# reesque/SfmFromScratch

Measured on AMD Instinct MI355X. Metric: images/sec detect+describe+match, 1080p, 1/2/4/8 MI355X, higher is better.
Workload: dtype f32; 1 GPU; BASELINE configs[1]: 32x 1080p per GPU, ScaleRotInvSIFT 4-level x2 octave pyramid, k=2500, fw 18, NNRatio 0.85 over consecutive pairs; frames_per_gpu=32, pairs_per_gpu=31, distinct_batches=2, parallelism=image-shard x1, batches_in_flight=2

## Files before the change

### include/sfmfeat.h

```cpp
#ifndef SFMFEAT_H_
#define SFMFEAT_H_

#include <stddef.h>
#include <stdint.h>

#ifdef __cplusplus
extern "C" {
#endif

#define SFM_OK 0
#define SFM_EINVAL 1
#define SFM_ESTATE 2
#define SFM_EDEVICE 3
#define SFM_ERANGE 4
#define SFM_EINDEX 5

#define SFM_MODE_SCALEROT 0
#define SFM_MODE_NAIVE 1

#define SFM_DESC_DIM 128
#define SFM_MAX_GAUSS 15
#define SFM_MAX_KSIZE 31
#define SFM_MAX_FW 64
#define SFM_MAX_LEVELS 12
// ... 221 lines not shown

int32_t sfm_debug_nms(int32_t device, const float* R, int32_t B, int32_t H, int32_t W, int32_t ksize,
                      const uint32_t* tnms, int32_t tile, uint64_t* keys_out, int64_t* counts_out);

#define SFM_SELECT_STATE_WORDS 11
#define SFM_SELECT_CONSTS 5
int32_t sfm_debug_select(int32_t device, int32_t nlevels, int32_t B, const float* const* R, const int32_t* H,
                         const int32_t* W, const int32_t* half_window, int32_t k, int32_t ksize, int64_t vmin,
                         int32_t force_exact, int32_t* x, int32_t* y, float* conf, int32_t* count,
                         uint32_t* state, int64_t* ncand, int32_t* consts);

float sfm_debug_time_harris(int32_t device, int32_t abl, int32_t B, int32_t H, int32_t W,
                            int32_t iters);
float sfm_debug_harris_stamps(int32_t device, int32_t abl, int32_t B, int32_t H, int32_t W,
                              int32_t iters, uint64_t* out, int64_t cap);

int64_t sfm_debug_match_stamps(uint64_t* out, int64_t cap);

int32_t sfm_debug_match_operands(sfm_ctx* ctx, int32_t slot, int64_t rows, uint16_t* hi, uint16_t* lo,
                                 float* norm2, float* rnorm, float* pmax);
int32_t sfm_debug_match_windows(sfm_ctx* ctx, int32_t pair, int64_t rows, int32_t* cand_n, float* cand_thr,
                                uint32_t* cand);
int32_t sfm_debug_match_skips(sfm_ctx* ctx, int32_t pair, int64_t rows, uint8_t* skip);

int32_t sfm_copy_wg(void* dst, const void* src, int64_t bytes, int32_t workgroups, void* stream);

int32_t sfm_debug_select_stats(sfm_ctx* ctx, int32_t* fallback_planes, int32_t* total_planes);
int32_t sfm_debug_pose_candidates(sfm_ctx* ctx, int32_t* cand_idx, int64_t entries);
int32_t sfm_debug_ransac_fits(sfm_ctx* ctx, double* F, int32_t* counts, int64_t entries);
int32_t sfm_debug_pnp_fits(sfm_ctx* ctx, double* hyp, int32_t* counts, double* start_Rt, int64_t entries);
int32_t sfm_debug_copy_level(sfm_ctx* ctx, int32_t l, int32_t what, float* out, void* stream);
int64_t sfm_debug_bmax_stride(int32_t h, int32_t w);
void sfm_debug_set_nms_blocks(int32_t mode);
int32_t sfm_debug_nms_blocks_rule(int32_t h, int32_t w, int32_t kcap, int32_t ksize);
int32_t sfm_debug_nms_blocks(int32_t device, const float* R, int32_t B, int32_t H, int32_t W, const uint32_t* tnms,
                             const uint32_t* fallback, int32_t blocks, int32_t inflate, uint64_t* keys_out,
                             int64_t* counts_out);


#ifdef __cplusplus
}
#endif

#endif
```

### sfmfromscratch_amd/_native.py

```python
from __future__ import annotations

import ctypes
import os
import sys
import threading

import numpy as np

from . import _abi
from ._abi import SfmParams

_HERE = os.path.dirname(os.path.abspath(__file__))
LIB_PATH = os.environ.get("SFMFEAT_LIB", os.path.join(_HERE, "lib", "libsfmfeat.so"))

_lib = None
_lib_lock = threading.Lock()

_fp = ctypes.POINTER(ctypes.c_float)
_i64p = ctypes.POINTER(ctypes.c_int64)
_i32p = ctypes.POINTER(ctypes.c_int32)
_u8p = ctypes.POINTER(ctypes.c_uint8)
_dp = ctypes.POINTER(ctypes.c_double)
_vp = ctypes.c_void_p

# ... 78 lines not shown
    "sfm_gate_destroy": (ctypes.c_int32, [_vp]),
    "sfm_ctx_set_gate": (ctypes.c_int32, [_vp, _vp]),
    "sfm_profile_enable": (ctypes.c_int32, [_vp, ctypes.c_int32]),
    "sfm_profile_stages": (ctypes.c_int32, [_vp, ctypes.c_int32]),
    "sfm_profile_read": (ctypes.c_int32, [_vp, ctypes.POINTER(ctypes.c_double), _i64p, ctypes.c_int32]),
    "sfm_profile_spans": (ctypes.c_int32, [_vp, ctypes.c_int64]),
    "sfm_profile_spans_read": (ctypes.c_int32, [_vp, _i64p, _i32p, ctypes.c_int64, _i64p, _i64p, ctypes.c_int32]),
    "sfm_debug_time_harris": (ctypes.c_float, [ctypes.c_int32] * 6),
    "sfm_debug_harris_stamps": (ctypes.c_float, [ctypes.c_int32] * 6 + [ctypes.c_void_p, ctypes.c_int64]),
    "sfm_debug_match_stamps": (ctypes.c_int64, [ctypes.c_void_p, ctypes.c_int64]),
    "sfm_debug_select_stats": (ctypes.c_int32, [_vp, _i32p, _i32p]),
    **_abi.MATCH_DEBUG_SIGNATURES,
    **_abi.GEOM_DEBUG_SIGNATURES,
    **_abi.SELECT_DEBUG_SIGNATURES,
    **_abi.PNP_DEBUG_SIGNATURES,
    "sfm_copy_wg": (ctypes.c_int32, [_vp, _vp, ctypes.c_int64, ctypes.c_int32, _vp]),
    "sfm_dist_unique_id": (ctypes.c_int32, [_u8p]),
    "sfm_dist_create": (ctypes.c_int32, [ctypes.c_int32, ctypes.c_int32, ctypes.c_int32, _u8p, ctypes.POINTER(_vp)]),
    "sfm_dist_destroy": (ctypes.c_int32, [_vp]),
    "sfm_dist_last_error": (ctypes.c_char_p, [_vp]),
    "sfm_dist_rank": (ctypes.c_int32, [_vp, _i32p, _i32p]),
    "sfm_dist_allgather_slots_dev": (ctypes.c_int32, [_vp, ctypes.c_int32, ctypes.c_int32, _vp, _vp, _vp, _vp, _vp,
                                                      _vp, ctypes.c_int64, _vp]),
    "sfm_dist_halo_dev": (ctypes.c_int32, [_vp, ctypes.c_int32, _vp, _vp, _vp, _vp, _vp, _vp, _vp]),

    "sfm_debug_copy_level": (ctypes.c_int32, [_vp, ctypes.c_int32, ctypes.c_int32, _vp, _vp]),
    "sfm_debug_atan2": (ctypes.c_int32, [ctypes.c_int32, _fp, _fp, _fp, ctypes.c_int64]),
    "sfm_debug_harris": (ctypes.c_int32, [ctypes.c_int32, _fp, ctypes.c_int32, ctypes.c_double, ctypes.c_int32,
                                          _fp, ctypes.c_int32, ctypes.c_int32, _fp, _fp, _i64p]),
    "sfm_debug_nms": (ctypes.c_int32, [ctypes.c_int32, _fp, ctypes.c_int32, ctypes.c_int32, ctypes.c_int32,
                                       ctypes.c_int32, _vp, ctypes.c_int32, _vp, _i64p]),
    "sfm_debug_bmax_stride": (ctypes.c_int64, [ctypes.c_int32, ctypes.c_int32]),
    "sfm_debug_set_nms_blocks": (None, [ctypes.c_int32]),
    "sfm_debug_nms_blocks_rule": (ctypes.c_int32, [ctypes.c_int32] * 4),
    "sfm_debug_nms_blocks": (ctypes.c_int32, [ctypes.c_int32, _fp, ctypes.c_int32, ctypes.c_int32, ctypes.c_int32,
                                              _vp, _vp, ctypes.c_int32, ctypes.c_int32, _vp, _i64p]),
}


class NativeLibraryMissing(ImportError):
    pass


def _preload_torch_hip_runtime():
    import importlib.util
    spec = importlib.util.find_spec("torch")
    if spec is None or not spec.submodule_search_locations:
        return
    for d in spec.submodule_search_locations:
        cand = os.path.join(d, "lib", "libamdhip64.so")
        if os.path.exists(cand):
            try:
                ctypes.CDLL(cand, mode=ctypes.RTLD_GLOBAL)
            except OSError:
                pass
            return


def _preload_torch_rccl():
    import importlib.util
    if "torch" not in sys.modules and importlib.util.find_spec("torch") is not None:
        import torch


def load_library(path: str | None = None):
    global _lib
# ... 444 lines not shown
    nc = ctypes.c_int64(0)
    check(load_library().sfm_debug_harris(device, g.ctypes.data_as(_fp), gs, params.alpha, params.ksize,
                                          img.ctypes.data_as(_fp), H, W, R.ctypes.data_as(_fp),
                                          med.ctypes.data_as(_fp), ctypes.byref(nc)))
    return R, med[0], nc.value


def debug_nms(R: np.ndarray, tnms, ksize: int = 3, tile: bool = False, device: int = 0):
    R = np.ascontiguousarray(R, dtype=np.float32)
    B, H, W = R.shape
    t = np.ascontiguousarray(tnms, dtype=np.uint32)
    keys = np.zeros(B * H * W, np.uint64)
    cnt = np.zeros(B, np.int64)
    check(load_library().sfm_debug_nms(device, R.ctypes.data_as(_fp), B, H, W, ksize, t.ctypes.data,
                                       int(tile), keys.ctypes.data, cnt.ctypes.data_as(_i64p)))
    return [np.sort(keys[b * H * W: b * H * W + cnt[b]]) for b in range(B)]


def debug_nms_blocks(R: np.ndarray, tnms, fallback=None, blocks: bool = True, inflate: bool = False, device: int = 0):
    R = np.ascontiguousarray(R, dtype=np.float32)
    B, H, W = R.shape
    t = np.ascontiguousarray(tnms, dtype=np.uint32)
    fb = np.zeros(B, np.uint32) if fallback is None else np.ascontiguousarray(fallback, dtype=np.uint32)
    assert t.shape == (B,) and fb.shape == (B,)
    keys = np.zeros(B * H * W, np.uint64)
    cnt = np.zeros(B, np.int64)
    check(load_library().sfm_debug_nms_blocks(device, R.ctypes.data_as(_fp), B, H, W, t.ctypes.data, fb.ctypes.data,
                                              int(blocks), int(inflate), keys.ctypes.data, cnt.ctypes.data_as(_i64p)))
    return [np.sort(keys[b * H * W: b * H * W + cnt[b]]) for b in range(B)]


def set_nms_blocks(mode: int):
    load_library().sfm_debug_set_nms_blocks(int(mode))


def nms_blocks_rule(h: int, w: int, kcap: int, ksize: int = 3) -> bool:
    return bool(load_library().sfm_debug_nms_blocks_rule(int(h), int(w), int(kcap), int(ksize)))


def bmax_stride(h: int, w: int) -> int:
    return int(load_library().sfm_debug_bmax_stride(int(h), int(w)))


def debug_geom(op: int, rows: np.ndarray, device: int = 0) -> np.ndarray:
    op = int(op)
    if not 0 <= op < len(_abi.GEOM_ROW_IN):
        raise ValueError(f"debug_geom: unknown op {op}")
    if not isinstance(rows, np.ndarray) or rows.dtype != np.float64 or not rows.flags.c_contiguous:
        raise ValueError("debug_geom: rows must be a C-contiguous float64 array")
    if rows.ndim != 2 or rows.shape[1] != _abi.GEOM_ROW_IN[op]:
        raise ValueError(f"debug_geom: op {op} takes rows of {_abi.GEOM_ROW_IN[op]} values, got shape {rows.shape}")
    n = rows.shape[0]
    if n > _abi.SFM_GEOM_MAX_ROWS:
        raise ValueError(f"debug_geom: at most {_abi.SFM_GEOM_MAX_ROWS} rows")
    out = np.empty((n, _abi.GEOM_ROW_OUT[op]), np.float64)
    if n:
        check(load_library().sfm_debug_geom(device, op, rows.ctypes.data, n, out.ctypes.data))
    return out


def select_constants(k: int) -> dict:
    consts = np.zeros(_abi.SFM_SELECT_CONSTS, np.int32)
    check(load_library().sfm_debug_select(0, 0, 0, None, None, None, None, int(k), 1, 0, 0, None, None, None, None,
                                          None, None, consts.ctypes.data))
    return dict(zip(_abi.SELECT_CONST_FIELDS, consts.tolist()))

# ... 147 lines not shown
```

### sfmfromscratch_amd/csrc/api_extract.hip

```cpp
#include "ctx.h"

using namespace sfm;

static_assert(kLayoutMedBins == kMedBins1 && kLayoutCounterStride == kCounterStride &&
                  kLayoutMedianStateBytes == sizeof(MedianState) && kLayoutSelectMaxLevels == kSelectMaxLevels,
              "extract_layout.h mirrors kernels.h");
static_assert(layout_bmax_stride(1080, 1920) == bmax_plane_stride(1080, 1920) &&
                  layout_bmax_stride(270, 480) == bmax_plane_stride(270, 480) &&
                  layout_bmax_stride(70, 132) == bmax_plane_stride(70, 132),
              "extract_layout.h mirrors kernels.h");

static int g_nms_blocks_override = -2;
void extract_set_nms_blocks(int mode) { g_nms_blocks_override = mode < -1 ? -2 : mode; }

LayoutSwitches extract_layout_switches() {
  LayoutSwitches s = extract_switches().layout;
  if (g_nms_blocks_override != -2) s.nms_blocks = g_nms_blocks_override;
  return s;
}

const ExtractSwitches& extract_switches() {
  static const ExtractSwitches sw = [] {
    ExtractSwitches s;
    s.layout.pyr_fused = env_int(getenv("SFMFEAT_PYR_FUSED"), 1) != 0;
    s.layout.exact_px = env_int(getenv("SFMFEAT_EXACT_PX"), 128);
    s.layout.select_merge = env_int(SFM_DIAG_ENV("SFMFEAT_SELECT_MERGE"), 1) != 0;
    s.layout.nms_blocks = env_int(SFM_DIAG_ENV("SFMFEAT_NMS_BLOCKS"), -1);
    s.fill_launches = env_int(SFM_DIAG_ENV("SFMFEAT_FILL_LAUNCHES"), 0) != 0;
    s.harris_group = env_int(SFM_DIAG_ENV("SFMFEAT_HARRIS_GROUP"), 0);
    s.gate_level = env_int(SFM_DIAG_ENV("SFMFEAT_GATE_LEVEL"), 0);
    s.select_caller = env_int(SFM_DIAG_ENV("SFMFEAT_SELECT_CALLER"), 0) == 1;
    s.skip = env_int(SFM_ABLATION_ENV("SFMFEAT_SKIP"), 0);
    return s;
  }();
  return sw;
}

namespace {

int layout_of(sfm_ctx* c, int B, int H, int W, ExtractLayout* y) {
  if (extract_layout(&c->p, c->kcap, B, H, W, c->serial, extract_layout_switches(), y) != SFM_OK)
    return set_err(c, SFM_EINVAL, "image too small for the pyramid");
  return SFM_OK;
}

int reserve(sfm_ctx* c, const ExtractLayout& y) {
  for (int i = 0; i < kExtractBufs; ++i)
    if (int rc = ensure(c, c->ex.buf[i], y.bytes[i])) return rc;
  return SFM_OK;
}

struct Extraction {
  sfm_ctx* c;
  const ExtractSwitches& sw;
  const ExtractLayout& y;
  int B, skip;
  hipStream_t st;
  int32_t* xy;
  float* desc;
  float* conf;
  int32_t* count;
  int64_t cap;
  MatchOperands mo;
  const float* lvl[SFM_MAX_LEVELS];
// ... 51 lines not shown
      q.scan = SelectScan{med(l), medcnt + y.counter[l], donecnt + y.counter[l], vmin, exact(l) ? 1 : 0};
      q.down[0] = q.down[1] = q.down[2] = nullptr;
      if (y.pyr_fused && l == 0)
        for (int k = 0; k < 3; ++k) q.down[k] = const_cast<float*>(lvl[1 + k]);
    }
    if (l1 - l0 == 1 && y.bmax[l0] >= 0 && ((uintptr_t)R(l0) & 15) == 0 &&
        nms_blocks_shape(y.lv[l0].w, c->p.ksize, 0) &&
        (extract_layout_switches().nms_blocks == 1 || harris_tiles_64(g, B, c->p.gaussian_size))) {
      g.l[0].bmax = bmax(l0);
      mapped[l0] = true;
      c->ex.last_mapped |= 1u << l0;
    }
    ProfilerWs& pr = c->prof;
    if (pr.span_cap > 0) {
      if (pr.span_n < pr.span_cap) {
        g.span = as<unsigned long long>(pr.spans) + 2 * pr.span_n++;
        pr.span_level.push_back(l0);
      } else {
        ++pr.span_dropped;
      }
    }
    const float alpha = (float)c->p.alpha;
    if (!(l0 > 0 && (skip & 16))) launch_harris_levels(g, B, as<float>(c->ex.gauss), c->p.gaussian_size, alpha, st);
  }

  void select_level(int l, hipStream_t s) {
    StageScope sc(c, SFM_PROF_TOPK, s);
    if (skip & 1) return;
    launch_select(R(l), cand(l), candcnt + y.counter[l], at<uint32_t>(kBufMedlist, y.sel[l]),
                  at<uint64_t>(kBufScratch, y.sel[l]), kp(l), std::max(c->kcap, 1), c->kcap, B, y.lv[l].h, y.lv[l].w,
                  c->p.ksize, y.lv[l].fw / 2, med(l), s);
  }

  void select_merged() {
    StageScope sc(c, SFM_PROF_TOPK, st);
    SelectLevels g{};
    g.n = y.L - y.L_aux;
    for (int l = y.L_aux; l < y.L; ++l)
      g.l[l - y.L_aux] = SelectLevels::Level{R(l), cand(l), candcnt + y.counter[l], at<uint32_t>(kBufMedlist, y.sel[l]),
                                             at<uint64_t>(kBufScratch, y.sel[l]), kp(l), med(l), y.lv[l].h, y.lv[l].w,
                                             y.lv[l].fw / 2};
    if (!(skip & 1)) launch_select_levels(g, std::max(c->kcap, 1), c->kcap, B, c->p.ksize, st);
  }

  void describe_level(int l, hipStream_t s) {
    StageScope sc(c, SFM_PROF_DESCRIBE, s);
    const int L = y.L;
    if ((skip & 2) && l != L - 1) {
      fused_ok = false;
      return;
    }
    bool ow = false;
    const bool r = launch_describe(lvl[l], B, y.lv[l].h, y.lv[l].w, y.lv[l].fw, c->p.mode == SFM_MODE_NAIVE ? 0 : 1,
                                   kp(l), c->kcap, as<int32_t>(c->ex.buf[kBufLc]), l, L, y.lv[l].scale, xy, desc, conf,
                                   cap, l == L - 1 ? count : nullptr, mo, &ow, s);
    if (l == L - 1) counted = r;
    fused_ok = fused_ok && ow;
  }

  int release_gate() {
    if (c->gate && !gate_released) {
      HIPCHK(c, hipEventRecord(c->gate->ev, st));
      c->gate->armed = true;
      gate_released = true;
    }
    return SFM_OK;
  }

  int run(const float* imgs);
};

int Extraction::run(const float* imgs) {
  const int L = y.L, L_aux = y.L_aux;
  CtxStreams& cs = c->s;
  int rc;
  lvl[0] = imgs;
  for (int l = 1; l < L; ++l) lvl[l] = at<float>(kBufLvl, y.lvl[l]);
  zeroed = sw.fill_launches;
  {
    StageScope sc(c, SFM_PROF_PYRAMID, st);
    if (!y.pyr_fused) pyramid_from(1);
  }
  if ((rc = operands_fused_begin(c, desc, count, cap, B, &mo))) return rc;
  if (mo.hi) HIPCHK(c, hipMemsetAsync(mo.pmax, 0, (size_t)B * match_pmax_bytes(mo.capP), st));
  fused_ok = mo.hi != nullptr;
  if (!zeroed || sw.fill_launches) {
    HIPCHK(c, hipMemsetAsync(c->ex.buf[kBufHist].p, 0, y.bytes[kBufHist], st));
    HIPCHK(c, hipMemsetAsync(c->ex.buf[kBufCounts].p, 0, y.bytes[kBufCounts], st));
    zeroed = true;
  }
  medcnt = as<unsigned long long>(c->ex.buf[kBufCounts]);
  candcnt = medcnt + y.counter_block;
  donecnt = medcnt + 3 * y.counter_block;
  hipStream_t ax = nullptr;
  if (L_aux > 0) {
    if (!cs.aux) HIPCHK(c, hipStreamCreateWithPriority(&cs.aux, hipStreamNonBlocking, cs.prio));
    ax = cs.aux;
    HIPCHK(c, hipEventRecord(cs.ev[L], st));
    HIPCHK(c, hipStreamWaitEvent(ax, cs.ev[L], 0));
  }
  for (int l0 = 0; l0 < L;) {
    int l1 = l0 + 1;
    if (sw.harris_group > 0 && l0 >= sw.harris_group) l1 = std::min(L, l0 + kHarrisMaxLevels);
    harris(l0, l1);
    if (y.pyr_fused && l0 == 0 && L > 4) {
      StageScope sc(c, SFM_PROF_PYRAMID, st);
      pyramid_from(4);
    }
    if (sw.gate_level >= l0 && sw.gate_level < l1 && (rc = release_gate())) return rc;
    for (int l = l0; l < l1; ++l) {
      if (!exact(l)) {
        StageScope sc(c, SFM_PROF_NMS, st);
        launch_nms(R(l), med(l), cand(l), candcnt + y.counter[l], B, y.lv[l].h, y.lv[l].w, c->p.ksize, 0, st, 0,
                   mapped[l] ? bmax(l) : nullptr);
      }
      if (l < L_aux) {
        if (sw.select_caller) select_level(l, st);
        HIPCHK(c, hipEventRecord(cs.ev[l], st));
        HIPCHK(c, hipStreamWaitEvent(ax, cs.ev[l], 0));
        if (!sw.select_caller) select_level(l, ax);
        if (l == L_aux - 1) HIPCHK(c, hipEventRecord(cs.ev[L + 2], ax));
        describe_level(l, ax);
      }
    }
    l0 = l1;
  }
  if ((rc = release_gate())) return rc;
  if (y.select_merged) {
    select_merged();
  } else {
    for (int l = L_aux; l < L; ++l) select_level(l, st);
  }
  if (L_aux > 0 && L > L_aux) HIPCHK(c, hipStreamWaitEvent(st, cs.ev[L + 2], 0));
  for (int l = L_aux; l < L; ++l) describe_level(l, st);
  if (L_aux > 0) {
    HIPCHK(c, hipEventRecord(cs.ev[L + 1], ax));
    HIPCHK(c, hipStreamWaitEvent(st, cs.ev[L + 1], 0));
  }
  if (!counted) launch_finalize_counts(as<int32_t>(c->ex.buf[kBufLc]), B, L, count, st);
  HIPCHK(c, hipGetLastError());
  if (fused_ok && counted) operands_fused_commit(c, B);
  return SFM_OK;
}

}

int extract_reserve(sfm_ctx* c, int B, int H, int W) {
  ExtractLayout y;
  if (int rc = layout_of(c, B, H, W, &y)) return rc;
  return reserve(c, y);
}

int extract_impl(sfm_ctx* c, const float* imgs, int B, int H, int W, int32_t* xy, float* desc, float* conf,
                 int32_t* count, int64_t cap, hipStream_t st) {
  if (B < 1 || H < 1 || W < 1) return set_err(c, SFM_EINVAL, "empty batch or image");
  if (cap < c->cap) return set_err(c, SFM_ERANGE, "slot capacity below L * int(k / L)");
  ExtractLayout y;
  int rc;
  if ((rc = layout_of(c, B, H, W, &y)) || (rc = reserve(c, y))) return rc;
  const ExtractSwitches& sw = extract_switches();
  ExtractWs& x = c->ex;
  const int skip = x.extractions++ > 0 ? sw.skip : 0;
  if (c->gate && c->gate->armed) HIPCHK(c, hipStreamWaitEvent(st, c->gate->ev, 0));
  x.last_B = B;
  x.last_H = H;
  x.last_W = W;
  x.last_mapped = 0;
// ... 79 lines not shown
```

### sfmfromscratch_amd/csrc/ctx.h

```cpp
#pragma once

#include <stdlib.h>
#include <string.h>

#include <algorithm>
#include <string>
#include <utility>
#include <vector>

#include "../../include/sfmfeat.h"
#include "extract_layout.h"
#include "kernels.h"

struct DevBuf {
  void* p = nullptr;
  size_t bytes = 0;
  DevBuf() = default;
  DevBuf(const DevBuf&) = delete;
  DevBuf& operator=(const DevBuf&) = delete;
  DevBuf(DevBuf&& o) noexcept : p(o.p), bytes(o.bytes) { o.p = nullptr, o.bytes = 0; }
  DevBuf& operator=(DevBuf&& o) noexcept {
    if (this != &o) {
      release();
      std::swap(p, o.p);
// ... 195 lines not shown
  hipStream_t st;
  hipEvent_t a = nullptr, b = nullptr;
  static hipEvent_t event(ProfilerWs& pr) {
    hipEvent_t e = nullptr;
    if (pr.pool.empty()) {
      (void)hipEventCreate(&e);
    } else {
      e = pr.pool.back();
      pr.pool.pop_back();
    }
    return e;
  }
  StageScope(sfm_ctx* c, int stage_, hipStream_t st_) : pr(c->prof), stage(stage_), st(st_) {
    if (pr.on && ((pr.mask >> stage) & 1u)) {
      a = event(pr);
      b = event(pr);
      (void)hipEventRecord(a, st);
    }
  }
  ~StageScope() {
    if (a) {
      (void)hipEventRecord(b, st);
      pr.pending.push_back({stage, {a, b}});
    }
  }
};

struct ExtractSwitches {
  sfm::LayoutSwitches layout;
  bool fill_launches;
  int harris_group;
  int gate_level;
  bool select_caller;
  int skip;
};
const ExtractSwitches& extract_switches();
sfm::LayoutSwitches extract_layout_switches();
void extract_set_nms_blocks(int mode);

int extract_reserve(sfm_ctx* c, int B, int H, int W);
int extract_impl(sfm_ctx* c, const float* imgs, int B, int H, int W, int32_t* xy, float* desc, float* conf,
                 int32_t* count, int64_t cap, hipStream_t st);

const std::vector<int32_t>& ransac_stream(sfm_ctx* c, int n, int iters);

int operands_fused_begin(sfm_ctx* c, const float* desc, const int32_t* count, int64_t cap, int B,
                         sfm::MatchOperands* mo);
void operands_fused_commit(sfm_ctx* c, int B);
void operands_fused_clear(sfm_ctx* c);
```

### sfmfromscratch_amd/csrc/debug_nms.hip

```cpp
#include <math.h>
#include <string.h>

#include <vector>

#include "ctx.h"

using namespace sfm;

extern "C" {

int64_t sfm_debug_bmax_stride(int32_t h, int32_t w) { return bmax_plane_stride(h, w); }

void sfm_debug_set_nms_blocks(int32_t mode) { extract_set_nms_blocks(mode); }

int32_t sfm_debug_nms_blocks_rule(int32_t h, int32_t w, int32_t kcap, int32_t ksize) {
  const LayoutSwitches sw;
  const bool exact = (int64_t)h * w < (int64_t)sw.exact_px * kcap;
  return nms_blocks_level(h, w, kcap, ksize, exact, -1) ? 1 : 0;
}

int32_t sfm_debug_nms_blocks(int32_t device, const float* R, int32_t B, int32_t H, int32_t W, const uint32_t* tnms,
                             const uint32_t* fallback, int32_t blocks, int32_t inflate, uint64_t* keys_out,
                             int64_t* counts_out) {
  if (!R || !tnms || !fallback || !keys_out || !counts_out || B < 1 || H < 1 || W < 4 || (W & 3)) return SFM_EINVAL;
  if (!nms_blocks_shape(W, 3, 0)) return SFM_EINVAL;
  if (hipSetDevice(device) != hipSuccess) return SFM_EDEVICE;
  const int64_t n = (int64_t)H * W, tot = n * B;
  const int MH = (H + 3) / 4, MW = W / 4;
  const int64_t stride = bmax_plane_stride(H, W);
  std::vector<float> M((size_t)B * stride, NAN);
  for (int b = 0; b < B; ++b)
    for (int by = 0; by < MH; ++by)
      for (int bx = 0; bx < MW; ++bx) {
        float m = -INFINITY;
        for (int i = 0; i < 4 && 4 * by + i < H; ++i)
          for (int e = 0; e < 4; ++e) m = fmaxf(m, R[(int64_t)b * n + (int64_t)(4 * by + i) * W + 4 * bx + e]);
        if (inflate) m = (by * MW + bx) % 3 == 0 ? INFINITY : nextafterf(m, INFINITY);
        M[(size_t)b * stride + (size_t)by * MW + bx] = m;
      }
  float *d_R = nullptr, *d_M = nullptr;
  MedianState* d_med = nullptr;
  unsigned long long* d_cnt = nullptr;
  uint64_t* d_cand = nullptr;
  int32_t rc = SFM_OK;
  if (hipMalloc(&d_R, tot * 4) || hipMalloc(&d_M, M.size() * 4) || hipMalloc(&d_med, sizeof(MedianState) * B) ||
      hipMalloc(&d_cnt, 8 * (size_t)B * kCounterStride) || hipMalloc(&d_cand, tot * 8)) {
// ... 31 lines not shown
```

### sfmfromscratch_amd/csrc/kernels.h

```cpp
#pragma once

#include <hip/hip_runtime.h>
#include <stdint.h>

#include <vector>

#include "common.h"

namespace sfm {

#define SFM_NMS_MAX_HALF 15

constexpr int kHistBits = 12;
constexpr int kHistBins = 1 << kHistBits;
constexpr int kMedBits1 = 11;
constexpr int kMedBins1 = 1 << kMedBits1;
constexpr int kTopkLdsCap = 8192;
constexpr int kMaxMatchRows = 16384;
constexpr int kMatchCandCap = 256;
constexpr int kCounterStride = 32;
constexpr int kMatchUnitPairBits = 20;

constexpr float kMatchScale = 256.0f;
constexpr float kMatchLoScale = 2048.0f;
// ... 385 lines not shown
    j1 = oj;
  } else {
    e2 = fminf(e2, o1);
  }
}
SFM_DEV RowBest top2_finish(float e1, int j1, float e2, float ratio) {
  RowBest rb;
  rb.col = -1;
  rb.nndr = 0.0f;
  const float d1 = sqrtf(e1), d2 = sqrtf(e2);
  if (d2 > 0.0f) {
    const float nndr = d1 / d2;
    if (nndr <= ratio) { rb.col = j1; rb.nndr = nndr; }
  }
  return rb;
}
void launch_transpose_desc(const float* desc, const int32_t* count, int nimg, int64_t cap,
                           int64_t capP, float* descT, hipStream_t st);
void launch_match_rows(const float* descT, const int32_t* count, int64_t capP, const int32_t* pairs,
                       int P, float ratio, RowBest* rows, int max_rows, hipStream_t st);
void launch_match_compact(const RowBest* rows, const int32_t* count, const int32_t* pairs, int P,
                          int max_rows, int64_t cap, int32_t* matches, float* conf, int32_t* nmatch,
                          int* reset_counter, hipStream_t st);
void init_match_attributes(int max_rows);
size_t match_pmax_bytes(int64_t capP);
void launch_match_prep(const float* desc, const int32_t* count, int nimg, int64_t cap, int64_t capP,
                       _Float16* hi, _Float16* lo, float* norm2, float* rnorm, void* pmax, hipStream_t st);
void launch_match_mfma(const float* desc, const int32_t* count, int64_t cap, int64_t capP,
                       const _Float16* hi, const _Float16* lo, const float* norm2, const float* rnorm,
                       const void* pmax, const int32_t* pairs, int P, float ratio,
                       RowBest* rows, int max_rows, uint32_t* cand, int32_t* cand_n, float* cand_thr,
                       uint8_t* cand_skip, uint32_t* work_list, int* ovf_count, int2* ovf_list, int32_t* units,
                       hipStream_t st);

}
```

### sfmfromscratch_amd/csrc/match_mfma.hip

```cpp
#include <stdlib.h>

#include <type_traits>

#include "kernels.h"

namespace sfm {

typedef _Float16 h8 __attribute__((ext_vector_type(8)));
typedef float f32x16 __attribute__((ext_vector_type(16)));

constexpr int kQW = 32;
constexpr int kWaves = 8;
constexpr int kQB = kQW * kWaves;
constexpr int kNT = 64 * kWaves;
constexpr int kRowH = 128 + 8;
constexpr int kCandCap = kMatchCandCap;
constexpr int kHalfCap = kCandCap / 2;
constexpr float kScale = kMatchScale;
constexpr float kLoScale = kMatchLoScale;

__global__ void __launch_bounds__(256) k_match_prep(const float* __restrict__ desc,
                                                   const int32_t* __restrict__ count, int64_t cap,
                                                   int64_t capP, _Float16* __restrict__ hi,
                                                   _Float16* __restrict__ lo,
// ... 611 lines not shown
  const float r2 = fminf(fmaxf(b1, ob1), fminf(b2, ob2));
  const float thr_final = fminf(r2 + E2, thr_w);
  const int ocnt = other_half(cnt);
  const bool unbounded = !(E2 <= 3.0e38f);
  bool todo = false;
  if (live && half == 0) {
    cand_thr[(int64_t)p * max_rows + qi] = thr_final;
    cand_n[(int64_t)p * max_rows + qi] = unbounded ? 0x7fff : cnt | (ocnt << 16);
    const bool over = cnt > kHalfCap || ocnt > kHalfCap || unbounded;
    if (over) {
      const int k = atomicAdd(ovf_count, 1);
      ovf_list[k] = make_int2(p, qi);
    }
    const bool skip = !over && proven_unmatched(fminf(b1, ob1), r2, E2, ratio);
    cand_skip[(int64_t)p * max_rows + qi] = skip ? 1 : 0;
    if (skip) {
      RowBest rb;
      rb.col = -1;
      rb.nndr = 0.0f;
      rows_out[(int64_t)p * max_rows + qi] = rb;
    }
    todo = !over && !skip;
  }
  const uint64_t bal = __ballot(todo);
  if (bal) {
    const int lead = __ffsll((unsigned long long)bal) - 1;
    int base = 0;
    if (lane == lead) base = atomicAdd(work_count, __popcll(bal));
    base = __shfl(base, lead);
    if (todo) work_list[base + __popcll(bal & ((1ull << lane) - 1ull))] = (uint32_t)(p * max_rows + qi);
  }
}

template <int ITEMS>
__global__ void __launch_bounds__(256) k_match_rerank(const float* __restrict__ desc,
                                                      const int32_t* __restrict__ count, int64_t cap,
                                                      const int32_t* __restrict__ pairs, int P, float ratio,
                                                      int max_rows, const uint32_t* __restrict__ cand,
                                                      const int32_t* __restrict__ cand_n,
                                                      const float* __restrict__ cand_thr,
                                                      const int* __restrict__ work_count,
                                                      const uint32_t* __restrict__ work_list,
                                                      RowBest* __restrict__ rows_out) {
  static_assert(ITEMS == 1 || ITEMS == 2, "one item per wavefront or per half-wave");
  constexpr int LPI = 64 / ITEMS;
  constexpr int GPI = LPI / 8;
  static_assert(kHalfCap % LPI == 0, "whole passes per half-list");
  __shared__ uint16_t sJ[4][ITEMS][kCandCap];
  const int lane = threadIdx.x & 63, wv = threadIdx.x >> 6, hf = lane / LPI, hl = lane % LPI;
  const int grp = hl >> 3, l8 = lane & 7;
  const int64_t t = ((int64_t)blockIdx.x * 4 + wv) * ITEMS + hf;
  bool ok = t < *work_count;
  if (!__any(ok)) return;
  const int64_t w = ok ? (int64_t)work_list[t] : 0;
  const int p = (int)(w / max_rows), row = (int)(w % max_rows);
  const int i1 = pairs[2 * p], i2 = pairs[2 * p + 1];
  int c0 = 0, c1 = 0;
  float thr = 0.0f;
  if (ok) {
    const int cw = cand_n[w];
    c0 = cw & 0xffff;
    c1 = cw >> 16;
    ok = c0 <= kHalfCap && c1 <= kHalfCap;
    thr = cand_thr[w];
  }
  const uint32_t* list = cand + w * kCandCap;
  const float* A = desc + ((int64_t)i1 * cap + row) * 128;
  const float* Bd = desc + (int64_t)i2 * cap * 128;
  float a[16];
#pragma unroll
  for (int i = 0; i < 16; ++i) a[i] = ok ? A[8 * i + l8] : 0.0f;
  int nk = 0;
  const uint64_t hmask = ITEMS == 1 ? ~0ull : hf ? 0xFFFFFFFF00000000ull : 0x00000000FFFFFFFFull;
  auto item_max = [](int v) { return ITEMS == 1 ? v : max(v, __shfl_xor(v, 32)); };
#pragma unroll
  for (int h = 0; h < 2; ++h) {
    const int ch = ok ? (h ? c1 : c0) : 0;
// ... 9 lines not shown
      nk += __popcll(bal);
    }
  }
  __builtin_amdgcn_wave_barrier();
  float e1 = INFINITY, e2 = INFINITY;
  int j1 = 0x7fffffff;
  const int nkmax = item_max(nk);
  for (int s0 = 0; s0 < nkmax; s0 += GPI) {
    const int sidx = s0 + grp;
    const bool okc = sidx < nk;
    const int j = okc ? (int)sJ[wv][hf][sidx] : 0;
    const float* b = Bd + (int64_t)j * 128;
    float r = 0.0f;
#pragma unroll
    for (int i = 0; i < 16; ++i) {
      const float dd = a[i] - b[8 * i + l8];
      const float sq = dd * dd;
      r = (i == 0) ? sq : r + sq;
    }
    r = r + __shfl_xor(r, 1);
    r = r + __shfl_xor(r, 2);
    r = r + __shfl_xor(r, 4);
    if (okc) top2_update(r, j, e1, j1, e2);
  }
#pragma unroll
  for (int off = 8; off < LPI; off <<= 1) {
    const float o1 = __shfl_xor(e1, off), o2 = __shfl_xor(e2, off);
    const int oj = __shfl_xor(j1, off);
    top2_merge(e1, j1, e2, o1, oj, o2);
  }
  if (hl == 0 && ok) rows_out[w] = top2_finish(e1, j1, e2, ratio);
}

__global__ void __launch_bounds__(256) k_match_overflow(const float* __restrict__ desc,
                                                        const int32_t* __restrict__ count, int64_t cap,
                                                        const int32_t* __restrict__ pairs, float ratio,
                                                        RowBest* __restrict__ rows_out, int max_rows,
                                                        const int* __restrict__ ovf_count,
                                                        const int2* __restrict__ ovf_list) {
  const int nov = *ovf_count;
  const int lane = threadIdx.x & 63;
  for (int w = blockIdx.x * 4 + (threadIdx.x >> 6); w < nov; w += gridDim.x * 4) {
    const int2 ent = ovf_list[w];
    const int p = ent.x, row = ent.y;
    const int i1 = pairs[2 * p], i2 = pairs[2 * p + 1];
    const int n2 = count[i2];
    const float* A = desc + ((int64_t)i1 * cap + row) * 128;
    const float* Bd = desc + (int64_t)i2 * cap * 128;
    float e1 = INFINITY, e2 = INFINITY;
    int j1 = 0x7fffffff;
    for (int j = lane; j < n2; j += 64) {
      const float dd = exact_sqdist(A, Bd + (int64_t)j * 128);
      top2_update(dd, j, e1, j1, e2);
    }
#pragma unroll
    for (int off = 32; off >= 1; off >>= 1) {
      const float o1 = __shfl_xor(e1, off), o2 = __shfl_xor(e2, off);
      const int oj = __shfl_xor(j1, off);
      top2_merge(e1, j1, e2, o1, oj, o2);
    }
    if (lane == 0) rows_out[(int64_t)p * max_rows + row] = top2_finish(e1, j1, e2, ratio);
  }
}

size_t match_units_words(int P, int max_rows) {
  return 1 + (size_t)P * ((max_rows + sweep_rows(3) - 1) / sweep_rows(3));
}

size_t match_pmax_bytes(int64_t capP) { return (size_t)(capP / kPrepRows) * sizeof(float2); }

void launch_match_prep(const float* desc, const int32_t* count, int nimg, int64_t cap, int64_t capP,
                       _Float16* hi, _Float16* lo, float* norm2, float* rnorm, void* pmax, hipStream_t st) {
  hipLaunchKernelGGL(k_match_prep, dim3((unsigned)(capP / kPrepRows), nimg), dim3(256), 0, st, desc, count, cap,
                     capP, hi, lo, norm2, rnorm, static_cast<float2*>(pmax));
}

void launch_match_mfma(const float* desc, const int32_t* count, int64_t cap, int64_t capP,
                       const _Float16* hi, const _Float16* lo, const float* norm2, const float* rnorm,
                       const void* pmax, const int32_t* pairs, int P, float ratio,
                       RowBest* rows, int max_rows, uint32_t* cand, int32_t* cand_n, float* cand_thr,
                       uint8_t* cand_skip, uint32_t* work_list, int* ovf_count, int2* ovf_list, int32_t* units,
                       hipStream_t st) {
  static const int stage = [] {
    const char* e = getenv("SFMFEAT_MATCH_STAGE");
    return (e && e[0] == 'r') ? 0 : (e && e[0] == '1') ? 1 : 3;
  }();
  static const bool use_units = [] {
    const char* e = SFM_DIAG_ENV("SFMFEAT_MATCH_UNITS");
    return !(e && e[0] == '0');
  }();
  int* const work_count = ovf_count + 1;
  const int qbr = stage == 3 ? sweep_rows(3) : kQB;
  const int qb = (max_rows + qbr - 1) / qbr;
  const dim3 grid((unsigned)(8 * ((P + 7) / 8) * qb));
  if (!use_units) units = nullptr;
  if (units)
    hipLaunchKernelGGL(k_match_units, dim3(1), dim3(1024), 0, st, count, pairs, P, max_rows, qbr, units, work_count);
  else
    (void)hipMemsetAsync(work_count, 0, sizeof(int), st);
#define SFM_SWEEP(A, ABL)                                                                             \
  hipLaunchKernelGGL((k_match_mfma<A, ABL>), grid, dim3(64 * sweep_waves(A)), 0, st, count, capP, hi, lo,  \
                     norm2, rnorm,                                                                         \
                     static_cast<const float2*>(pmax), pairs, P, max_rows, cand, cand_n, cand_thr, ovf_count, \
                     ovf_list, units, ratio, cand_skip, rows, work_count, work_list)
  static const int abl = [] {
    const char* e = SFM_ABLATION_ENV("SFMFEAT_MATCH_ABL");
    return e ? atoi(e) : 0;
  }();
#ifdef SFM_ABLATIONS
  switch (abl) {
    case 1: SFM_SWEEP(1, 1); break;
    case 2: SFM_SWEEP(1, 2); break;
    case 3: SFM_SWEEP(1, 3); break;
    case 4: SFM_SWEEP(1, 4); break;
    case 6: SFM_SWEEP(1, 6); break;
    case 16: SFM_SWEEP(1, 16); break;
    case 17: SFM_SWEEP(1, 17); break;
    case 32: SFM_SWEEP(1, 32); break;
    default: if (stage == 0) SFM_SWEEP(0, 0); else if (stage == 3) SFM_SWEEP(3, 0); else SFM_SWEEP(1, 0);
  }
#else
  (void)abl;
  if (stage == 0)
    SFM_SWEEP(0, 0);
  else if (stage == 3)
    SFM_SWEEP(3, 0);
  else
    SFM_SWEEP(1, 0);
#endif
#undef SFM_SWEEP
  static const int rr2 = [] {
    const char* e = getenv("SFMFEAT_RERANK2");
    return e ? atoi(e) : 1;
  }();
  if (rr2)
    hipLaunchKernelGGL(k_match_rerank<2>, dim3((unsigned)(((int64_t)P * max_rows + 7) / 8)), dim3(256), 0, st, desc,
                       count, cap, pairs, P, ratio, max_rows, cand, cand_n, cand_thr, work_count,
                       work_list, rows);
  else
    hipLaunchKernelGGL(k_match_rerank<1>, dim3((unsigned)(((int64_t)P * max_rows + 3) / 4)), dim3(256), 0, st, desc,
                       count, cap, pairs, P, ratio, max_rows, cand, cand_n, cand_thr, work_count,
                       work_list, rows);
  hipLaunchKernelGGL(k_match_overflow, dim3(256), dim3(256), 0, st, desc, count, cap, pairs, ratio, rows, max_rows,
                     ovf_count, ovf_list);
}

int64_t match_stamps_copy(uint64_t* out, int64_t cap) {
#ifdef SFM_ABLATIONS
  const int64_t n1 = (int64_t)sizeof(g_match_stamps) / 8, n = n1 + (int64_t)sizeof(g_match_wg) / 8;
  if (cap < n) return -1;
  if (hipMemcpyFromSymbol(out, HIP_SYMBOL(g_match_stamps), sizeof(g_match_stamps)) != hipSuccess) return -1;
  if (hipMemcpyFromSymbol(out + n1, HIP_SYMBOL(g_match_wg), sizeof(g_match_wg)) != hipSuccess) return -1;
  return n;
#else
  (void)out;
  (void)cap;
  return -1;
#endif
}

}
```

Baseline: 45560 images/sec.

## Add optional fused overflow tail in rerank and aux-stream extract tail scheduling

Adds an option to run the match overflow rows inside the rerank kernel as extra trailing blocks, using a wider 8-lane-per-candidate distance loop instead of a separate launch. Adds an option to move one more extract level's select and describe onto the auxiliary stream, so it overlaps with the merged selection of the remaining levels. Caps rerank VGPRs at 52 to raise occupancy, at the risk of register spills. Both schedule options default off and are exposed through env vars and debug setters.

```diff
diff --git a/include/sfmfeat.h b/include/sfmfeat.h
--- a/include/sfmfeat.h
+++ b/include/sfmfeat.h
@@ -277,6 +277,8 @@
 int32_t sfm_debug_copy_level(sfm_ctx* ctx, int32_t l, int32_t what, float* out, void* stream);
 int64_t sfm_debug_bmax_stride(int32_t h, int32_t w);
 void sfm_debug_set_nms_blocks(int32_t mode);
+void sfm_debug_set_tail_schedule(int32_t mode);
+void sfm_debug_set_match_tail(int32_t mode);
 int32_t sfm_debug_nms_blocks_rule(int32_t h, int32_t w, int32_t kcap, int32_t ksize);
 int32_t sfm_debug_nms_blocks(int32_t device, const float* R, int32_t B, int32_t H, int32_t W, const uint32_t* tnms,
                              const uint32_t* fallback, int32_t blocks, int32_t inflate, uint64_t* keys_out,
diff --git a/sfmfromscratch_amd/_native.py b/sfmfromscratch_amd/_native.py
--- a/sfmfromscratch_amd/_native.py
+++ b/sfmfromscratch_amd/_native.py
@@ -134,6 +134,8 @@
                                        ctypes.c_int32, _vp, ctypes.c_int32, _vp, _i64p]),
     "sfm_debug_bmax_stride": (ctypes.c_int64, [ctypes.c_int32, ctypes.c_int32]),
     "sfm_debug_set_nms_blocks": (None, [ctypes.c_int32]),
+    "sfm_debug_set_tail_schedule": (None, [ctypes.c_int32]),
+    "sfm_debug_set_match_tail": (None, [ctypes.c_int32]),
     "sfm_debug_nms_blocks_rule": (ctypes.c_int32, [ctypes.c_int32] * 4),
     "sfm_debug_nms_blocks": (ctypes.c_int32, [ctypes.c_int32, _fp, ctypes.c_int32, ctypes.c_int32, ctypes.c_int32,
                                               _vp, _vp, ctypes.c_int32, ctypes.c_int32, _vp, _i64p]),
@@ -644,6 +646,14 @@
 
 def set_nms_blocks(mode: int):
     load_library().sfm_debug_set_nms_blocks(int(mode))
+
+
+def set_tail_schedule(mode: int):
+    load_library().sfm_debug_set_tail_schedule(int(mode))
+
+
+def set_match_tail(mode: int):
+    load_library().sfm_debug_set_match_tail(int(mode))
 
 
 def nms_blocks_rule(h: int, w: int, kcap: int, ksize: int = 3) -> bool:
diff --git a/sfmfromscratch_amd/csrc/api_extract.hip b/sfmfromscratch_amd/csrc/api_extract.hip
--- a/sfmfromscratch_amd/csrc/api_extract.hip
+++ b/sfmfromscratch_amd/csrc/api_extract.hip
@@ -12,6 +12,9 @@
 
 static int g_nms_blocks_override = -2;
 void extract_set_nms_blocks(int mode) { g_nms_blocks_override = mode < -1 ? -2 : mode; }
+
+static int g_tail_aux_override = -2;
+void extract_set_tail_aux(int mode) { g_tail_aux_override = (mode == 0 || mode == 1) ? mode : -2; }
 
 LayoutSwitches extract_layout_switches() {
   LayoutSwitches s = extract_switches().layout;
@@ -30,6 +33,7 @@
     s.harris_group = env_int(SFM_DIAG_ENV("SFMFEAT_HARRIS_GROUP"), 0);
     s.gate_level = env_int(SFM_DIAG_ENV("SFMFEAT_GATE_LEVEL"), 0);
     s.select_caller = env_int(SFM_DIAG_ENV("SFMFEAT_SELECT_CALLER"), 0) == 1;
+    s.tail_aux = env_int(SFM_DIAG_ENV("SFMFEAT_TAIL_AUX"), 0) != 0;
     s.skip = env_int(SFM_ABLATION_ENV("SFMFEAT_SKIP"), 0);
     return s;
   }();
@@ -147,14 +151,15 @@
                   c->p.ksize, y.lv[l].fw / 2, med(l), s);
   }
 
-  void select_merged() {
+  void select_merged(int from) {
+    if (y.L - from == 1) return select_level(from, st);
     StageScope sc(c, SFM_PROF_TOPK, st);
     SelectLevels g{};
-    g.n = y.L - y.L_aux;
-    for (int l = y.L_aux; l < y.L; ++l)
-      g.l[l - y.L_aux] = SelectLevels::Level{R(l), cand(l), candcnt + y.counter[l], at<uint32_t>(kBufMedlist, y.sel[l]),
-                                             at<uint64_t>(kBufScratch, y.sel[l]), kp(l), med(l), y.lv[l].h, y.lv[l].w,
-                                             y.lv[l].fw / 2};
+    g.n = y.L - from;
+    for (int l = from; l < y.L; ++l)
+      g.l[l - from] = SelectLevels::Level{R(l), cand(l), candcnt + y.counter[l], at<uint32_t>(kBufMedlist, y.sel[l]),
+                                          at<uint64_t>(kBufScratch, y.sel[l]), kp(l), med(l), y.lv[l].h, y.lv[l].w,
+                                          y.lv[l].fw / 2};
     if (!(skip & 1)) launch_select_levels(g, std::max(c->kcap, 1), c->kcap, B, c->p.ksize, st);
   }
 
@@ -214,6 +219,8 @@
     HIPCHK(c, hipEventRecord(cs.ev[L], st));
     HIPCHK(c, hipStreamWaitEvent(ax, cs.ev[L], 0));
   }
+  const int tail_aux = g_tail_aux_override != -2 ? g_tail_aux_override : (int)sw.tail_aux;
+  const int L_fork = L_aux + (L_aux > 0 && y.select_merged && L - L_aux >= 2 && tail_aux ? 1 : 0);
   for (int l0 = 0; l0 < L;) {
     int l1 = l0 + 1;
     if (sw.harris_group > 0 && l0 >= sw.harris_group) l1 = std::min(L, l0 + kHarrisMaxLevels);
@@ -229,12 +236,12 @@
         launch_nms(R(l), med(l), cand(l), candcnt + y.counter[l], B, y.lv[l].h, y.lv[l].w, c->p.ksize, 0, st, 0,
                    mapped[l] ? bmax(l) : nullptr);
       }
-      if (l < L_aux) {
+      if (l < L_fork) {
         if (sw.select_caller) select_level(l, st);
         HIPCHK(c, hipEventRecord(cs.ev[l], st));
         HIPCHK(c, hipStreamWaitEvent(ax, cs.ev[l], 0));
         if (!sw.select_caller) select_level(l, ax);
-        if (l == L_aux - 1) HIPCHK(c, hipEventRecord(cs.ev[L + 2], ax));
+        if (l == L_fork - 1) HIPCHK(c, hipEventRecord(cs.ev[L + 2], ax));
         describe_level(l, ax);
       }
     }
@@ -242,12 +249,12 @@
   }
   if ((rc = release_gate())) return rc;
   if (y.select_merged) {
-    select_merged();
+    select_merged(L_fork);
   } else {
-    for (int l = L_aux; l < L; ++l) select_level(l, st);
-  }
-  if (L_aux > 0 && L > L_aux) HIPCHK(c, hipStreamWaitEvent(st, cs.ev[L + 2], 0));
-  for (int l = L_aux; l < L; ++l) describe_level(l, st);
+    for (int l = L_fork; l < L; ++l) select_level(l, st);
+  }
+  if (L_aux > 0 && L > L_fork) HIPCHK(c, hipStreamWaitEvent(st, cs.ev[L + 2], 0));
+  for (int l = L_fork; l < L; ++l) describe_level(l, st);
   if (L_aux > 0) {
     HIPCHK(c, hipEventRecord(cs.ev[L + 1], ax));
     HIPCHK(c, hipStreamWaitEvent(st, cs.ev[L + 1], 0));
diff --git a/sfmfromscratch_amd/csrc/ctx.h b/sfmfromscratch_amd/csrc/ctx.h
--- a/sfmfromscratch_amd/csrc/ctx.h
+++ b/sfmfromscratch_amd/csrc/ctx.h
@@ -251,11 +251,13 @@
   int harris_group;
   int gate_level;
   bool select_caller;
+  bool tail_aux;
   int skip;
 };
 const ExtractSwitches& extract_switches();
 sfm::LayoutSwitches extract_layout_switches();
 void extract_set_nms_blocks(int mode);
+void extract_set_tail_aux(int mode);
 
 int extract_reserve(sfm_ctx* c, int B, int H, int W);
 int extract_impl(sfm_ctx* c, const float* imgs, int B, int H, int W, int32_t* xy, float* desc, float* conf,
diff --git a/sfmfromscratch_amd/csrc/debug_nms.hip b/sfmfromscratch_amd/csrc/debug_nms.hip
--- a/sfmfromscratch_amd/csrc/debug_nms.hip
+++ b/sfmfromscratch_amd/csrc/debug_nms.hip
@@ -12,6 +12,10 @@
 int64_t sfm_debug_bmax_stride(int32_t h, int32_t w) { return bmax_plane_stride(h, w); }
 
 void sfm_debug_set_nms_blocks(int32_t mode) { extract_set_nms_blocks(mode); }
+
+void sfm_debug_set_tail_schedule(int32_t mode) { extract_set_tail_aux(mode); }
+
+void sfm_debug_set_match_tail(int32_t mode) { match_set_ovf_launch(mode == 0 ? 1 : mode == 1 ? 0 : -2); }
 
 int32_t sfm_debug_nms_blocks_rule(int32_t h, int32_t w, int32_t kcap, int32_t ksize) {
   const LayoutSwitches sw;
diff --git a/sfmfromscratch_amd/csrc/kernels.h b/sfmfromscratch_amd/csrc/kernels.h
--- a/sfmfromscratch_amd/csrc/kernels.h
+++ b/sfmfromscratch_amd/csrc/kernels.h
@@ -441,5 +441,6 @@
                        RowBest* rows, int max_rows, uint32_t* cand, int32_t* cand_n, float* cand_thr,
                        uint8_t* cand_skip, uint32_t* work_list, int* ovf_count, int2* ovf_list, int32_t* units,
                        hipStream_t st);
-
-}
+void match_set_ovf_launch(int mode);
+
+}
diff --git a/sfmfromscratch_amd/csrc/match_mfma.hip b/sfmfromscratch_amd/csrc/match_mfma.hip
--- a/sfmfromscratch_amd/csrc/match_mfma.hip
+++ b/sfmfromscratch_amd/csrc/match_mfma.hip
@@ -667,8 +667,84 @@
   }
 }
 
+__global__ void __launch_bounds__(256) k_match_overflow(const float* __restrict__ desc,
+                                                        const int32_t* __restrict__ count, int64_t cap,
+                                                        const int32_t* __restrict__ pairs, float ratio,
+                                                        RowBest* __restrict__ rows_out, int max_rows,
+                                                        const int* __restrict__ ovf_count,
+                                                        const int2* __restrict__ ovf_list) {
+  const int nov = *ovf_count;
+  const int lane = threadIdx.x & 63;
+  for (int w = blockIdx.x * 4 + (threadIdx.x >> 6); w < nov; w += gridDim.x * 4) {
+    const int2 ent = ovf_list[w];
+    const int p = ent.x, row = ent.y;
+    const int i1 = pairs[2 * p], i2 = pairs[2 * p + 1];
+    const int n2 = count[i2];
+    const float* A = desc + ((int64_t)i1 * cap + row) * 128;
+    const float* Bd = desc + (int64_t)i2 * cap * 128;
+    float e1 = INFINITY, e2 = INFINITY;
+    int j1 = 0x7fffffff;
+    for (int j = lane; j < n2; j += 64) {
+      const float dd = exact_sqdist(A, Bd + (int64_t)j * 128);
+      top2_update(dd, j, e1, j1, e2);
+    }
+#pragma unroll
+    for (int off = 32; off >= 1; off >>= 1) {
+      const float o1 = __shfl_xor(e1, off), o2 = __shfl_xor(e2, off);
+      const int oj = __shfl_xor(j1, off);
+      top2_merge(e1, j1, e2, o1, oj, o2);
+    }
+    if (lane == 0) rows_out[(int64_t)p * max_rows + row] = top2_finish(e1, j1, e2, ratio);
+  }
+}
+
+SFM_DEV void overflow_rows_wide(const float* __restrict__ desc, const int32_t* __restrict__ count, int64_t cap,
+                                const int32_t* __restrict__ pairs, float ratio, RowBest* __restrict__ rows_out,
+                                int max_rows, const int* __restrict__ ovf_count, const int2* __restrict__ ovf_list,
+                                int blk, int nblk) {
+  const int nov = *ovf_count;
+  const int lane = threadIdx.x & 63, grp = lane >> 3, l8 = lane & 7;
+  for (int w = blk * 4 + (threadIdx.x >> 6); w < nov; w += nblk * 4) {
+    const int2 ent = ovf_list[w];
+    const int p = ent.x, row = ent.y;
+    const int i1 = pairs[2 * p], i2 = pairs[2 * p + 1];
+    const int n2 = count[i2];
+    const float* A = desc + ((int64_t)i1 * cap + row) * 128;
+    const float* Bd = desc + (int64_t)i2 * cap * 128;
+    float a[16];
+#pragma unroll
+    for (int i = 0; i < 16; ++i) a[i] = A[8 * i + l8];
+    float e1 = INFINITY, e2 = INFINITY;
+    int j1 = 0x7fffffff;
+    for (int j0 = 0; j0 < n2; j0 += 8) {
+      const int j = j0 + grp;
+      const bool okc = j < n2;
+      const float* b = Bd + (int64_t)(okc ? j : 0) * 128;
+      float r = 0.0f;
+#pragma unroll
+      for (int i = 0; i < 16; ++i) {
+        const float dd = a[i] - b[8 * i + l8];
+        const float sq = dd * dd;
+        r = (i == 0) ? sq : r + sq;
+      }
+      r = r + __shfl_xor(r, 1);
+      r = r + __shfl_xor(r, 2);
+      r = r + __shfl_xor(r, 4);
+      if (okc) top2_update(r, j, e1, j1, e2);
+    }
+#pragma unroll
+    for (int off = 8; off < 64; off <<= 1) {
+      const float o1 = __shfl_xor(e1, off), o2 = __shfl_xor(e2, off);
+      const int oj = __shfl_xor(j1, off);
+      top2_merge(e1, j1, e2, o1, oj, o2);
+    }
+    if (lane == 0) rows_out[(int64_t)p * max_rows + row] = top2_finish(e1, j1, e2, ratio);
+  }
+}
+
 template <int ITEMS>
-__global__ void __launch_bounds__(256) k_match_rerank(const float* __restrict__ desc,
+__global__ void __launch_bounds__(256) __attribute__((amdgpu_num_vgpr(52)))
+k_match_rerank(const float* __restrict__ desc,
                                                       const int32_t* __restrict__ count, int64_t cap,
                                                       const int32_t* __restrict__ pairs, int P, float ratio,
                                                       int max_rows, const uint32_t* __restrict__ cand,
@@ -676,8 +752,15 @@
                                                       const float* __restrict__ cand_thr,
                                                       const int* __restrict__ work_count,
                                                       const uint32_t* __restrict__ work_list,
-                                                      RowBest* __restrict__ rows_out) {
+                                                      RowBest* __restrict__ rows_out, int rr_blocks,
+                                                      const int* __restrict__ ovf_count,
+                                                      const int2* __restrict__ ovf_list) {
   static_assert(ITEMS == 1 || ITEMS == 2, "one item per wavefront or per half-wave");
+  if ((int)blockIdx.x >= rr_blocks) {
+    overflow_rows_wide(desc, count, cap, pairs, ratio, rows_out, max_rows, ovf_count, ovf_list,
+                       (int)blockIdx.x - rr_blocks, (int)gridDim.x - rr_blocks);
+    return;
+  }
   constexpr int LPI = 64 / ITEMS;
   constexpr int GPI = LPI / 8;
   static_assert(kHalfCap % LPI == 0, "whole passes per half-list");
@@ -753,37 +836,6 @@
   if (hl == 0 && ok) rows_out[w] = top2_finish(e1, j1, e2, ratio);
 }
 
-__global__ void __launch_bounds__(256) k_match_overflow(const float* __restrict__ desc,
-                                                        const int32_t* __restrict__ count, int64_t cap,
-                                                        const int32_t* __restrict__ pairs, float ratio,
-                                                        RowBest* __restrict__ rows_out, int max_rows,
-                                                        const int* __restrict__ ovf_count,
-                                                        const int2* __restrict__ ovf_list) {
-  const int nov = *ovf_count;
-  const int lane = threadIdx.x & 63;
-  for (int w = blockIdx.x * 4 + (threadIdx.x >> 6); w < nov; w += gridDim.x * 4) {
-    const int2 ent = ovf_list[w];
-    const int p = ent.x, row = ent.y;
-    const int i1 = pairs[2 * p], i2 = pairs[2 * p + 1];
-    const int n2 = count[i2];
-    const float* A = desc + ((int64_t)i1 * cap + row) * 128;
-    const float* Bd = desc + (int64_t)i2 * cap * 128;
-    float e1 = INFINITY, e2 = INFINITY;
-    int j1 = 0x7fffffff;
-    for (int j = lane; j < n2; j += 64) {
-      const float dd = exact_sqdist(A, Bd + (int64_t)j * 128);
-      top2_update(dd, j, e1, j1, e2);
-    }
-#pragma unroll
-    for (int off = 32; off >= 1; off >>= 1) {
-      const float o1 = __shfl_xor(e1, off), o2 = __shfl_xor(e2, off);
-      const int oj = __shfl_xor(j1, off);
-      top2_merge(e1, j1, e2, o1, oj, o2);
-    }
-    if (lane == 0) rows_out[(int64_t)p * max_rows + row] = top2_finish(e1, j1, e2, ratio);
-  }
-}
-
 size_t match_units_words(int P, int max_rows) {
   return 1 + (size_t)P * ((max_rows + sweep_rows(3) - 1) / sweep_rows(3));
 }
@@ -795,6 +847,8 @@
   hipLaunchKernelGGL(k_match_prep, dim3((unsigned)(capP / kPrepRows), nimg), dim3(256), 0, st, desc, count, cap,
                      capP, hi, lo, norm2, rnorm, static_cast<float2*>(pmax));
 }
+
+static int g_ovf_launch_override = -2;
 
 void launch_match_mfma(const float* desc, const int32_t* count, int64_t cap, int64_t capP,
                        const _Float16* hi, const _Float16* lo, const float* norm2, const float* rnorm,
@@ -854,17 +908,25 @@
     const char* e = getenv("SFMFEAT_RERANK2");
     return e ? atoi(e) : 1;
   }();
+  constexpr int kOvfBlocks = 256;
+  static const bool ovf_launch_env = env_int(SFM_DIAG_ENV("SFMFEAT_MATCH_OVF_LAUNCH"), 1) != 0;
+  const bool ovf_launch = g_ovf_launch_override != -2 ? g_ovf_launch_override != 0 : ovf_launch_env;
+  const int tail = ovf_launch ? 0 : kOvfBlocks;
+  const int rr_blocks = (int)(((int64_t)P * max_rows + (rr2 ? 7 : 3)) / (rr2 ? 8 : 4));
   if (rr2)
-    hipLaunchKernelGGL(k_match_rerank<2>, dim3((unsigned)(((int64_t)P * max_rows + 7) / 8)), dim3(256), 0, st, desc,
-                       count, cap, pairs, P, ratio, max_rows, cand, cand_n, cand_thr, work_count,
-                       work_list, rows);
+    hipLaunchKernelGGL(k_match_rerank<2>, dim3((unsigned)(rr_blocks + tail)), dim3(256), 0, st, desc, count, cap, pairs,
+                       P, ratio, max_rows, cand, cand_n, cand_thr, work_count, work_list, rows, rr_blocks, ovf_count,
+                       ovf_list);
   else
-    hipLaunchKernelGGL(k_match_rerank<1>, dim3((unsigned)(((int64_t)P * max_rows + 3) / 4)), dim3(256), 0, st, desc,
-                       count, cap, pairs, P, ratio, max_rows, cand, cand_n, cand_thr, work_count,
-                       work_list, rows);
-  hipLaunchKernelGGL(k_match_overflow, dim3(256), dim3(256), 0, st, desc, count, cap, pairs, ratio, rows, max_rows,
-                     ovf_count, ovf_list);
-}
+    hipLaunchKernelGGL(k_match_rerank<1>, dim3((unsigned)(rr_blocks + tail)), dim3(256), 0, st, desc, count, cap, pairs,
+                       P, ratio, max_rows, cand, cand_n, cand_thr, work_count, work_list, rows, rr_blocks, ovf_count,
+                       ovf_list);
+  if (ovf_launch)
+    hipLaunchKernelGGL(k_match_overflow, dim3(kOvfBlocks), dim3(256), 0, st, desc, count, cap, pairs, ratio, rows,
+                       max_rows, ovf_count, ovf_list);
+}
+
+void match_set_ovf_launch(int mode) { g_ovf_launch_override = (mode == 0 || mode == 1) ? mode : -2; }
 
 int64_t match_stamps_copy(uint64_t* out, int64_t cap) {
 #ifdef SFM_ABLATIONS
```

Result: slower. 45000 images/sec (-1.2%).
